# Azure/mmlspark

Measured on NVIDIA H100. Metric: boosting_iters_per_sec, higher is better.
Workload: dtype int64 fixed-point histograms over u8 bins (fp32 gradients, fp64 split gains)

## Files before the change

### mmlspark_b200/csrc/hist_kernel.cuh

```cuda
#pragma once
#include <cstdint>
#include <cuda_runtime.h>
#include <cub/block/block_scan.cuh>

namespace b200gbm {

constexpr int kTileFeat = 32;
constexpr int kBins = 256;
constexpr int kLoBits = 18;
constexpr int kFlushRows = 1 << (32 - kLoBits);
#ifndef B200GBM_K4_EXPERIMENT
#define B200GBM_K4_EXPERIMENT 0
#endif
constexpr int kPlaneWords = kBins * kTileFeat;

struct HistWork {
  int begin;
  int count;
  int use_idx;
  int buf;
};

__global__ void __launch_bounds__(256)
k_gather_q(const HistWork* __restrict__ work, const int* __restrict__ idx0, const int* __restrict__ idx1, const int4* __restrict__ qgh,
           int4* __restrict__ qord) {
  const HistWork w = *work;
  if (!w.use_idx) return;
  const int* __restrict__ idx = w.buf ? idx1 : idx0;
  for (int i = blockIdx.x * blockDim.x + threadIdx.x; i < w.count; i += gridDim.x * blockDim.x) {
    const int p = w.begin + i;
    qord[p] = qgh[idx[p]];
  }
}

constexpr int kBoundBlockRows = 4096;
struct RowBlockBound {
  const int* prefix;
  int blocks;
};
inline int bound_blocks(int num_data) { return (num_data + kBoundBlockRows - 1) / kBoundBlockRows; }

__global__ void __launch_bounds__(256)
k_block_maxcnt(const uint8_t* __restrict__ bins, size_t rows_stride, int num_data, int num_columns, int* __restrict__ prefix) {
  __shared__ unsigned cnt[kBins * kTileFeat];
  __shared__ unsigned wmax[8];
  const int tile = blockIdx.y, tid = threadIdx.x;
  for (int e = tid; e < kBins * kTileFeat; e += blockDim.x) cnt[e] = 0u;
  __syncthreads();
  const int r0 = blockIdx.x * kBoundBlockRows, rows = min(kBoundBlockRows, num_data - r0);
  const unsigned* wp = reinterpret_cast<const unsigned*>(bins + (static_cast<size_t>(tile) * rows_stride + r0) * kTileFeat);
  for (int e = tid; e < rows * 8; e += blockDim.x) {
    const unsigned word = wp[e];
    const int c0 = (e & 7) * 4, rot = (e >> 3) & 3;
#pragma unroll
    for (int k = 0; k < 4; ++k) {
      const int kk = (k + rot) & 3;
      atomicAdd(&cnt[((word >> (8 * kk)) & 0xFFu) * kTileFeat + c0 + kk], 1u);
    }
  }
  __syncthreads();
  const int ncol = min(kTileFeat, num_columns - tile * kTileFeat);
  unsigned m = 0u;
  for (int e = tid; e < kBins * kTileFeat; e += blockDim.x)
    if ((e & (kTileFeat - 1)) < ncol) m = max(m, cnt[e]);
  m = __reduce_max_sync(0xffffffffu, m);
  if ((tid & 31) == 0) wmax[tid >> 5] = m;
  __syncthreads();
  if (tid == 0) {
    for (int i = 1; i < static_cast<int>(blockDim.x >> 5); ++i) m = max(m, wmax[i]);
    prefix[static_cast<size_t>(tile) * (gridDim.x + 1) + blockIdx.x] = static_cast<int>(m);
  }
}

__global__ void __launch_bounds__(1024) k_block_bound_prefix(int blocks, int* __restrict__ prefix) {
  using Scan = cub::BlockScan<int, 1024>;
  __shared__ typename Scan::TempStorage tmp;
  int* p = prefix + static_cast<size_t>(blockIdx.x) * (blocks + 1);
  int carry = 0;
  for (int b0 = 0; b0 < blocks; b0 += 1024) {
    const int b = b0 + threadIdx.x;
    const int v = b < blocks ? p[b] : 0;
    int ex, total;
    Scan(tmp).ExclusiveSum(v, ex, total);
    if (b < blocks) p[b] = carry + ex;
    carry += total;
    __syncthreads();
  }
  if (threadIdx.x == 0) p[blocks] = carry;
}

inline void launch_block_bound(const uint8_t* bins, size_t rows_stride, int num_data, int num_tiles, int num_columns, int* prefix,
                               cudaStream_t stream) {
  const int blocks = bound_blocks(num_data);
  if (blocks > 0) k_block_maxcnt<<<dim3(blocks, num_tiles), 256, 0, stream>>>(bins, rows_stride, num_data, num_columns, prefix);
  k_block_bound_prefix<<<num_tiles, 1024, 0, stream>>>(blocks, prefix);
}


__device__ __forceinline__ void cp_async16(void* smem, const void* gmem, bool valid) {
  unsigned s = static_cast<unsigned>(__cvta_generic_to_shared(smem));
  int sz = valid ? 16 : 0;
  asm volatile("cp.async.cg.shared.global [%0], [%1], 16, %2;\n" ::"r"(s), "l"(gmem), "r"(sz));
}
template <int N>
__device__ __forceinline__ void cp_async_wait() {
  asm volatile("cp.async.wait_group %0;\n" ::"n"(N));
}

constexpr int kWsConsumerWarps = 16;
constexpr int kWsProducerWarps = 2;
constexpr int kWsThreads = (kWsConsumerWarps + kWsProducerWarps) * 32;
constexpr int kWsStageRows = 512;
constexpr int kWsStages = 3;
constexpr int kFlushSlabBins = 32;
constexpr int kFlushRowBytes = kFlushSlabBins * 16;
constexpr int kFlushStageBytes = kTileFeat * kFlushRowBytes;
constexpr int kWsSmemBytes = 4 * kPlaneWords * 4 + kWsStages * (kWsStageRows * 32 + kWsStageRows * 16) + kFlushStageBytes + 64;
static_assert(kWsSmemBytes <= 227 * 1024, "K4 shared memory exceeds the 227 KB per block of sm_90");
static_assert(kFlushSlabBins * kTileFeat == 2 * kWsConsumerWarps * 32, "a flush slab is two (g,h) pairs per consumer thread");

__device__ __forceinline__ unsigned smem_u32(const void* p) { return static_cast<unsigned>(__cvta_generic_to_shared(p)); }
__device__ __forceinline__ void mbar_init(unsigned long long* bar, unsigned count) {
  asm volatile("mbarrier.init.shared::cta.b64 [%0], %1;\n" ::"r"(smem_u32(bar)), "r"(count));
}
__device__ __forceinline__ void mbar_arrive(unsigned long long* bar) {
  asm volatile("mbarrier.arrive.shared::cta.b64 _, [%0];\n" ::"r"(smem_u32(bar)) : "memory");
}
__device__ __forceinline__ void mbar_arrive_expect_tx(unsigned long long* bar, unsigned bytes) {
  asm volatile("mbarrier.arrive.expect_tx.shared::cta.b64 _, [%0], %1;\n" ::"r"(smem_u32(bar)), "r"(bytes) : "memory");
}
__device__ __forceinline__ void mbar_expect_tx(unsigned long long* bar, unsigned bytes) {
  asm volatile("mbarrier.expect_tx.relaxed.cta.shared::cta.b64 [%0], %1;\n" ::"r"(smem_u32(bar)), "r"(bytes) : "memory");
}
__device__ __forceinline__ void mbar_wait(unsigned long long* bar, unsigned parity) {
  asm volatile(
      "{\n"
      ".reg .pred p;\n"
      "WAIT_LOOP:\n"
      "mbarrier.try_wait.parity.shared::cta.b64 p, [%0], %1;\n"
      "@p bra DONE;\n"
      "bra WAIT_LOOP;\n"
      "DONE:\n"
      "}\n" ::"r"(smem_u32(bar)), "r"(parity) : "memory");
}
__device__ __forceinline__ void tma_bulk_g2s(void* smem_dst, const void* gmem_src, unsigned bytes, unsigned long long* bar) {
  asm volatile("cp.async.bulk.shared::cluster.global.mbarrier::complete_tx::bytes [%0], [%1], %2, [%3];\n" ::"r"(smem_u32(smem_dst)),
               "l"(gmem_src), "r"(bytes), "r"(smem_u32(bar))
               : "memory");
}
__device__ __forceinline__ void cp_async_mbar_arrive_noinc(unsigned long long* bar) {
  asm volatile("cp.async.mbarrier.arrive.noinc.shared::cta.b64 [%0];\n" ::"r"(smem_u32(bar)) : "memory");
}
__device__ __forceinline__ void bulk_reduce_add_u64(unsigned long long* gmem_dst, const void* smem_src, unsigned bytes) {
  asm volatile("cp.reduce.async.bulk.global.shared::cta.bulk_group.add.u64 [%0], [%1], %2;\n" ::"l"(gmem_dst), "r"(smem_u32(smem_src)),
               "r"(bytes)
               : "memory");
}
__device__ __forceinline__ void bulk_commit() { asm volatile("cp.async.bulk.commit_group;\n" ::: "memory"); }
__device__ __forceinline__ void bulk_wait_read_all() { asm volatile("cp.async.bulk.wait_group.read 0;\n" ::: "memory"); }
__device__ __forceinline__ void bulk_wait_all() { asm volatile("cp.async.bulk.wait_group 0;\n" ::: "memory"); }
__device__ __forceinline__ void fence_proxy_async_smem() { asm volatile("fence.proxy.async.shared::cta;\n" ::: "memory"); }

template <int NATOM>
__global__ void __launch_bounds__(kWsThreads, 1)
k4_hist_build_ws(const uint8_t* __restrict__ bins, size_t rows_stride, int num_tiles, const int4* __restrict__ qgh,
                 const int4* __restrict__ qord, const int* __restrict__ idx0, const int* __restrict__ idx1,
                 const HistWork* __restrict__ work, unsigned long long* __restrict__ hist, RowBlockBound bound) {
  extern __shared__ __align__(128) unsigned char smem_raw[];
  unsigned* plane = reinterpret_cast<unsigned*>(smem_raw);
  unsigned char* stage_bins = smem_raw + 4 * kPlaneWords * 4;
  int4* stage_q = reinterpret_cast<int4*>(stage_bins + kWsStages * kWsStageRows * 32);
  unsigned char* flush_stage = reinterpret_cast<unsigned char*>(stage_q) + kWsStages * kWsStageRows * 16;
  unsigned long long* full_bar = reinterpret_cast<unsigned long long*>(flush_stage + kFlushStageBytes);
  unsigned long long* empty_bar = full_bar + kWsStages;

  const HistWork w = *work;
  const int n = w.count;
  if (n <= 0) return;
  const int tid = threadIdx.x, lane = tid & 31, warp = tid >> 5;
  const int* __restrict__ idx = w.buf ? idx1 : idx0;

  long long cells_rows = static_cast<long long>(n) * num_tiles;
  int rpi = static_cast<int>((cells_rows + 4LL * gridDim.x - 1) / (4LL * gridDim.x));
  rpi = (rpi + kWsStageRows - 1) / kWsStageRows * kWsStageRows;
  rpi = max(rpi, kWsStageRows);
  rpi = min(rpi, kFlushRows);
  const int chunks = (n + rpi - 1) / rpi;
  const long long items = static_cast<long long>(chunks) * num_tiles;
  const int i0 = static_cast<int>(items * blockIdx.x / gridDim.x);
  const int i1 = static_cast<int>(items * (blockIdx.x + 1) / gridDim.x);
  if (i0 >= i1) return;

  if (tid == 0) {
    for (int i = 0; i < kWsStages; ++i) { mbar_init(&full_bar[i], kWsProducerWarps * 32); mbar_init(&empty_bar[i], kWsConsumerWarps); }
    asm volatile("fence.mbarrier_init.release.cluster;\n" ::: "memory");
  }
  for (int e = tid; e < 4 * kPlaneWords; e += kWsThreads) plane[e] = 0u;
  __syncthreads();

  unsigned gs = 0;
  if (warp >= kWsConsumerWarps) {
    const int ptid = tid - kWsConsumerWarps * 32;
    constexpr int kPT = kWsProducerWarps * 32;
    constexpr int kPerLane = kWsStageRows / kPT;
    for (int item = i0; item < i1; ++item) {
      const int tile = item / chunks, chunk = item - tile * chunks;
      const int row0 = chunk * rpi;
      const int nrows = min(rpi, n - row0);
      const int nst = (nrows + kWsStageRows - 1) / kWsStageRows;
      const uint8_t* tbins = bins + static_cast<size_t>(tile) * rows_stride * 32;
      for (int s = 0; s < nst; ++s, ++gs) {
        const int slot = gs % kWsStages;
        mbar_wait(&empty_bar[slot], ((gs / kWsStages) & 1u) ^ 1u);
        const int p0 = row0 + s * kWsStageRows;
        const int rows = min(kWsStageRows, row0 + nrows - p0);
        unsigned char* db = stage_bins + slot * kWsStageRows * 32;
        int4* dq = stage_q + slot * kWsStageRows;
        if (!w.use_idx) {
          if (ptid == 0) {
            mbar_arrive_expect_tx(&full_bar[slot], static_cast<unsigned>(rows) * 48u);
            const size_t r = static_cast<size_t>(w.begin + p0);
            tma_bulk_g2s(db, tbins + r * 32, static_cast<unsigned>(rows) * 32u, &full_bar[slot]);
            tma_bulk_g2s(dq, qgh + r, static_cast<unsigned>(rows) * 16u, &full_bar[slot]);
          } else {
            mbar_arrive(&full_bar[slot]);
          }
        } else {
          const int* ip = idx + w.begin + p0;
          if (ptid == 0) {
            mbar_expect_tx(&full_bar[slot], static_cast<unsigned>(rows) * 16u);
            tma_bulk_g2s(dq, qord + static_cast<size_t>(w.begin + p0), static_cast<unsigned>(rows) * 16u, &full_bar[slot]);
          }
          int rr[2 * kPerLane];
#pragma unroll
          for (int k = 0; k < 2 * kPerLane; ++k) { const int j = (ptid + k * kPT) >> 1; rr[k] = j < rows ? ip[j] : -1; }
#pragma unroll
          for (int k = 0; k < 2 * kPerLane; ++k) {
            const int hh = ptid + k * kPT, j = hh >> 1, half = (hh & 1) * 16;
            if (rr[k] >= 0) cp_async16(db + j * 32 + half, tbins + static_cast<size_t>(rr[k]) * 32 + half, true);
          }
          cp_async_mbar_arrive_noinc(&full_bar[slot]);
        }
      }
    }
    cp_async_wait<0>();
  } else {
#if B200GBM_K4_EXPERIMENT >= 1 && B200GBM_K4_EXPERIMENT <= 3
    unsigned exp_sink = 0;
#endif
    const int sub = lane >> 2, rot = lane & 3;
    auto item_rows = [&](int it, int& first, int& last) {
      const int t = it / chunks, r0 = (it - t * chunks) * rpi;
      first = w.begin + r0;
      last = first + min(rpi, n - r0) - 1;
      if (w.use_idx && bound.prefix) { first = idx[first]; last = idx[last]; }
    };
    auto item_bound = [&](int it, int first, int last) -> int {
      const int t = it / chunks, nr = min(rpi, n - (it - t * chunks) * rpi);
      if (!bound.prefix) return nr;
      const int* p = bound.prefix + static_cast<size_t>(t) * (bound.blocks + 1);
      return min(nr, p[last / kBoundBlockRows + 1] - p[first / kBoundBlockRows]);
    };
    int first, last;
    item_rows(i0, first, last);
    int next_bound = item_bound(i0, first, last);
    if (i0 + 1 < i1) item_rows(i0 + 1, first, last);
    int acc_bound = 0;
    for (int item = i0; item < i1; ++item) {
      const int tile = item / chunks, chunk = item - tile * chunks;
      const int row0 = chunk * rpi;
      const int nrows = min(rpi, n - row0);
      const int nst = (nrows + kWsStageRows - 1) / kWsStageRows;
      acc_bound += next_bound;
      next_bound = 0;
      if (item + 1 < i1) {
        next_bound = item_bound(item + 1, first, last);
        if (item + 2 < i1) item_rows(item + 2, first, last);
      }
      for (int s = 0; s < nst; ++s, ++gs) {
        const int slot = gs % kWsStages;
        mbar_wait(&full_bar[slot], (gs / kWsStages) & 1u);
        const int rows = min(kWsStageRows, nrows - s * kWsStageRows);
        const unsigned* sw = reinterpret_cast<const unsigned*>(stage_bins + slot * kWsStageRows * 32);
        const int4* sq = stage_q + slot * kWsStageRows;
        const int groups = (rows + 31) >> 5;
        for (int g = warp; g < groups; g += kWsConsumerWarps) {
          const int r = g * 32 + lane;
          if (r < rows) {
            const int4 q = sq[r];
            const unsigned* rw = sw + r * 8;
#pragma unroll
            for (int k = 0; k < 8; ++k) {
              const int w8 = (sub + k) & 7;
              const unsigned word = rw[w8];
#pragma unroll
              for (int j = 0; j < 4; ++j) {
                const int kk = (j + rot) & 3;
                const unsigned b = (word >> (8 * kk)) & 0xFFu;
                const unsigned a = b * 32u + static_cast<unsigned>(w8 * 4 + kk);
#if B200GBM_K4_EXPERIMENT == 0 || B200GBM_K4_EXPERIMENT == 4
                atomicAdd(&plane[a], static_cast<unsigned>(q.x));
                atomicAdd(&plane[kPlaneWords + a], static_cast<unsigned>(q.y));
                atomicAdd(&plane[2 * kPlaneWords + a], static_cast<unsigned>(q.z));
                if (NATOM == 4) atomicAdd(&plane[3 * kPlaneWords + a], static_cast<unsigned>(q.w));
#else
                if (B200GBM_K4_EXPERIMENT >= 2) atomicAdd(&plane[a], static_cast<unsigned>(q.x));
                if (B200GBM_K4_EXPERIMENT >= 3) atomicAdd(&plane[kPlaneWords + a], static_cast<unsigned>(q.y));
                if (B200GBM_K4_EXPERIMENT == 1) exp_sink ^= a + static_cast<unsigned>(q.x ^ q.y ^ q.z ^ q.w);
#endif
              }
            }
          }
        }
#if B200GBM_K4_EXPERIMENT >= 1 && B200GBM_K4_EXPERIMENT <= 3
        if (exp_sink == 0x12345679u) plane[lane] = exp_sink;
#endif
        __syncwarp();
        if (lane == 0) mbar_arrive(&empty_bar[slot]);
      }
      const bool flush = (item + 1 == i1) || ((item + 1) / chunks != tile) || (acc_bound + next_bound > kFlushRows);
      if (!flush) continue;
      acc_bound = 0;
      asm volatile("bar.sync 1, %0;\n" ::"n"(kWsConsumerWarps * 32) : "memory");
      unsigned long long* htile = hist + static_cast<size_t>(tile) * kTileFeat * kBins * 2;
      int sbin[2];
#pragma unroll
      for (int i = 0; i < 2; ++i) sbin[i] = (warp + i * kWsConsumerWarps + lane) & (kFlushSlabBins - 1);
      for (int b0 = 0; b0 < kBins; b0 += kFlushSlabBins) {
        long long g[2], h[2];
        bool nz = false;
#pragma unroll
        for (int i = 0; i < 2; ++i) {
          const int e = (b0 + sbin[i]) * kTileFeat + lane;
          const unsigned ghi = plane[e], glo = plane[kPlaneWords + e], hhi = plane[2 * kPlaneWords + e];
          const unsigned hlo = (NATOM == 4) ? plane[3 * kPlaneWords + e] : 0u;
          plane[e] = 0u;
          plane[kPlaneWords + e] = 0u;
          plane[2 * kPlaneWords + e] = 0u;
          if (NATOM == 4) plane[3 * kPlaneWords + e] = 0u;
          nz |= (ghi | glo | hhi | hlo) != 0u;
          g[i] = (static_cast<long long>(static_cast<int>(ghi)) << kLoBits) + static_cast<long long>(glo);
          h[i] = (NATOM == 4) ? (static_cast<long long>(static_cast<int>(hhi)) << kLoBits) + static_cast<long long>(hlo)
                              : static_cast<long long>(hhi);
        }
        if (tid == 0) bulk_wait_read_all();
        asm volatile("bar.sync 1, %0;\n" ::"n"(kWsConsumerWarps * 32) : "memory");
#pragma unroll
        for (int i = 0; i < 2; ++i)
          *reinterpret_cast<longlong2*>(flush_stage + lane * kFlushRowBytes + sbin[i] * 16) = make_longlong2(g[i], h[i]);
        fence_proxy_async_smem();
        int any;
        asm volatile(
            "{\n"
            ".reg .pred p, q;\n"
            "setp.ne.u32 p, %1, 0;\n"
            "bar.red.or.pred q, 1, %2, p;\n"
            "selp.s32 %0, 1, 0, q;\n"
            "}\n"
            : "=r"(any)
            : "r"(static_cast<unsigned>(nz)), "n"(kWsConsumerWarps * 32)
            : "memory");
#if B200GBM_K4_EXPERIMENT != 4
        if (tid == 0 && any) {
          for (int f = 0; f < kTileFeat; ++f)
            bulk_reduce_add_u64(htile + (static_cast<size_t>(f) * kBins + b0) * 2, flush_stage + f * kFlushRowBytes, kFlushSlabBins * 16);
          bulk_commit();
        }
#else
        (void)any; (void)htile;
#endif
      }
    }
    if (tid == 0) bulk_wait_all();
  }
}

inline cudaError_t set_k4_smem_limit() {
  const cudaError_t e = cudaFuncSetAttribute(k4_hist_build_ws<4>, cudaFuncAttributeMaxDynamicSharedMemorySize, kWsSmemBytes);
  if (e != cudaSuccess) return e;
  return cudaFuncSetAttribute(k4_hist_build_ws<3>, cudaFuncAttributeMaxDynamicSharedMemorySize, kWsSmemBytes);
}

inline void launch_k4(bool const_hessian, const uint8_t* bins, size_t rows_stride, int num_tiles, const int4* qgh, const int4* qord,
                      const int* idx0, const int* idx1, const HistWork* work, unsigned long long* hist, RowBlockBound bound, int grid,
                      cudaStream_t stream) {
  if (const_hessian)
    k4_hist_build_ws<3><<<grid, kWsThreads, kWsSmemBytes, stream>>>(bins, rows_stride, num_tiles, qgh, qord, idx0, idx1, work, hist, bound);
  else
    k4_hist_build_ws<4><<<grid, kWsThreads, kWsSmemBytes, stream>>>(bins, rows_stride, num_tiles, qgh, qord, idx0, idx1, work, hist, bound);
}

}
```

Measured before the change: 6.325.

## Band CTAs by row range across tiles and add L2 evict-first hints on bin loads

Work assignment in the warp-specialized histogram kernel changes: when each CTA has enough rows, CTAs are grouped into row bands so that all feature tiles for a row range are processed together by a set of CTAs. This keeps the shared gradient/hessian rows hot in L2 across tiles. Bin loads (TMA bulk and cp.async) now carry an L2 evict_first cache policy so streamed bin bytes do not displace the reused gradient data. An experiment-5 path that aliases the gradient source is also added behind a macro that is off by default. The new partitioning adds index math and may worsen load balance for tail CTAs.

```diff
diff --git a/mmlspark_b200/csrc/hist_kernel.cuh b/mmlspark_b200/csrc/hist_kernel.cuh
--- a/mmlspark_b200/csrc/hist_kernel.cuh
+++ b/mmlspark_b200/csrc/hist_kernel.cuh
@@ -97,10 +97,14 @@
 }
 
 
-__device__ __forceinline__ void cp_async16(void* smem, const void* gmem, bool valid) {
+__device__ __forceinline__ unsigned long long l2_evict_first_policy() {
+  unsigned long long p;
+  asm volatile("createpolicy.fractional.L2::evict_first.b64 %0, 1.0;\n" : "=l"(p));
+  return p;
+}
+__device__ __forceinline__ void cp_async16(void* smem, const void* gmem, unsigned long long l2_policy) {
   unsigned s = static_cast<unsigned>(__cvta_generic_to_shared(smem));
-  int sz = valid ? 16 : 0;
-  asm volatile("cp.async.cg.shared.global [%0], [%1], 16, %2;\n" ::"r"(s), "l"(gmem), "r"(sz));
+  asm volatile("cp.async.cg.shared.global.L2::cache_hint [%0], [%1], 16, %2;\n" ::"r"(s), "l"(gmem), "l"(l2_policy));
 }
 template <int N>
 __device__ __forceinline__ void cp_async_wait() {
@@ -146,6 +150,12 @@
 __device__ __forceinline__ void tma_bulk_g2s(void* smem_dst, const void* gmem_src, unsigned bytes, unsigned long long* bar) {
   asm volatile("cp.async.bulk.shared::cluster.global.mbarrier::complete_tx::bytes [%0], [%1], %2, [%3];\n" ::"r"(smem_u32(smem_dst)),
                "l"(gmem_src), "r"(bytes), "r"(smem_u32(bar))
+               : "memory");
+}
+__device__ __forceinline__ void tma_bulk_g2s_hint(void* smem_dst, const void* gmem_src, unsigned bytes, unsigned long long* bar,
+                                                  unsigned long long l2_policy) {
+  asm volatile("cp.async.bulk.shared::cluster.global.mbarrier::complete_tx::bytes.L2::cache_hint [%0], [%1], %2, [%3], %4;\n"
+               ::"r"(smem_u32(smem_dst)), "l"(gmem_src), "r"(bytes), "r"(smem_u32(bar)), "l"(l2_policy)
                : "memory");
 }
 __device__ __forceinline__ void cp_async_mbar_arrive_noinc(unsigned long long* bar) {
@@ -180,16 +190,42 @@
   const int tid = threadIdx.x, lane = tid & 31, warp = tid >> 5;
   const int* __restrict__ idx = w.buf ? idx1 : idx0;
 
-  long long cells_rows = static_cast<long long>(n) * num_tiles;
-  int rpi = static_cast<int>((cells_rows + 4LL * gridDim.x - 1) / (4LL * gridDim.x));
+  const int num_ctas = static_cast<int>(gridDim.x), band_ctas = num_ctas / num_tiles * num_tiles;
+  const long long per_cta = static_cast<long long>(n) * num_tiles / num_ctas;
+  int seg_begin = 0, seg_end = n, seg_ctas = num_ctas, seg_cta = blockIdx.x;
+  if (band_ctas > 0 && per_cta >= kFlushRows) {
+    const int bands = band_ctas / num_tiles;
+    const bool tail = band_ctas < num_ctas;
+    const long long band_rows = tail ? per_cta : (n + bands - 1LL) / bands;
+    const int nb = tail ? static_cast<int>(bands * band_rows) : n;
+    if (seg_cta < band_ctas) {
+      const int r = seg_cta / num_tiles;
+      seg_begin = static_cast<int>(min(r * band_rows, static_cast<long long>(nb)));
+      seg_end = static_cast<int>(min(seg_begin + band_rows, static_cast<long long>(nb)));
+      seg_ctas = num_tiles;
+      seg_cta -= r * num_tiles;
+    } else {
+      seg_begin = nb;
+      seg_ctas = num_ctas - band_ctas;
+      seg_cta -= band_ctas;
+    }
+  }
+  const int seg_rows = seg_end - seg_begin;
+  const long long cells_rows = static_cast<long long>(seg_rows) * num_tiles;
+  int rpi = static_cast<int>((cells_rows + 4LL * seg_ctas - 1) / (4LL * seg_ctas));
   rpi = (rpi + kWsStageRows - 1) / kWsStageRows * kWsStageRows;
   rpi = max(rpi, kWsStageRows);
   rpi = min(rpi, kFlushRows);
-  const int chunks = (n + rpi - 1) / rpi;
+  const int chunks = (seg_rows + rpi - 1) / rpi;
   const long long items = static_cast<long long>(chunks) * num_tiles;
-  const int i0 = static_cast<int>(items * blockIdx.x / gridDim.x);
-  const int i1 = static_cast<int>(items * (blockIdx.x + 1) / gridDim.x);
+  const int i0 = static_cast<int>(items * seg_cta / seg_ctas);
+  const int i1 = static_cast<int>(items * (seg_cta + 1) / seg_ctas);
   if (i0 >= i1) return;
+  auto item_span = [&](int it, int& tile, int& row0, int& nrows) {
+    tile = it / chunks;
+    row0 = seg_begin + (it - tile * chunks) * rpi;
+    nrows = min(rpi, seg_end - row0);
+  };
 
   if (tid == 0) {
     for (int i = 0; i < kWsStages; ++i) { mbar_init(&full_bar[i], kWsProducerWarps * 32); mbar_init(&empty_bar[i], kWsConsumerWarps); }
@@ -203,10 +239,10 @@
     const int ptid = tid - kWsConsumerWarps * 32;
     constexpr int kPT = kWsProducerWarps * 32;
     constexpr int kPerLane = kWsStageRows / kPT;
+    const unsigned long long bins_policy = l2_evict_first_policy();
     for (int item = i0; item < i1; ++item) {
-      const int tile = item / chunks, chunk = item - tile * chunks;
-      const int row0 = chunk * rpi;
-      const int nrows = min(rpi, n - row0);
+      int tile, row0, nrows;
+      item_span(item, tile, row0, nrows);
       const int nst = (nrows + kWsStageRows - 1) / kWsStageRows;
       const uint8_t* tbins = bins + static_cast<size_t>(tile) * rows_stride * 32;
       for (int s = 0; s < nst; ++s, ++gs) {
@@ -220,8 +256,12 @@
           if (ptid == 0) {
             mbar_arrive_expect_tx(&full_bar[slot], static_cast<unsigned>(rows) * 48u);
             const size_t r = static_cast<size_t>(w.begin + p0);
-            tma_bulk_g2s(db, tbins + r * 32, static_cast<unsigned>(rows) * 32u, &full_bar[slot]);
+            tma_bulk_g2s_hint(db, tbins + r * 32, static_cast<unsigned>(rows) * 32u, &full_bar[slot], bins_policy);
+#if B200GBM_K4_EXPERIMENT == 5
+            tma_bulk_g2s(dq, qgh + (p0 & 65535), static_cast<unsigned>(rows) * 16u, &full_bar[slot]);
+#else
             tma_bulk_g2s(dq, qgh + r, static_cast<unsigned>(rows) * 16u, &full_bar[slot]);
+#endif
           } else {
             mbar_arrive(&full_bar[slot]);
           }
@@ -229,7 +269,11 @@
           const int* ip = idx + w.begin + p0;
           if (ptid == 0) {
             mbar_expect_tx(&full_bar[slot], static_cast<unsigned>(rows) * 16u);
+#if B200GBM_K4_EXPERIMENT == 5
+            tma_bulk_g2s(dq, qord + (p0 & 65535), static_cast<unsigned>(rows) * 16u, &full_bar[slot]);
+#else
             tma_bulk_g2s(dq, qord + static_cast<size_t>(w.begin + p0), static_cast<unsigned>(rows) * 16u, &full_bar[slot]);
+#endif
           }
           int rr[2 * kPerLane];
 #pragma unroll
@@ -237,7 +281,7 @@
 #pragma unroll
           for (int k = 0; k < 2 * kPerLane; ++k) {
             const int hh = ptid + k * kPT, j = hh >> 1, half = (hh & 1) * 16;
-            if (rr[k] >= 0) cp_async16(db + j * 32 + half, tbins + static_cast<size_t>(rr[k]) * 32 + half, true);
+            if (rr[k] >= 0) cp_async16(db + j * 32 + half, tbins + static_cast<size_t>(rr[k]) * 32 + half, bins_policy);
           }
           cp_async_mbar_arrive_noinc(&full_bar[slot]);
         }
@@ -250,13 +294,15 @@
 #endif
     const int sub = lane >> 2, rot = lane & 3;
     auto item_rows = [&](int it, int& first, int& last) {
-      const int t = it / chunks, r0 = (it - t * chunks) * rpi;
+      int t, r0, nr;
+      item_span(it, t, r0, nr);
       first = w.begin + r0;
-      last = first + min(rpi, n - r0) - 1;
+      last = first + nr - 1;
       if (w.use_idx && bound.prefix) { first = idx[first]; last = idx[last]; }
     };
     auto item_bound = [&](int it, int first, int last) -> int {
-      const int t = it / chunks, nr = min(rpi, n - (it - t * chunks) * rpi);
+      int t, r0, nr;
+      item_span(it, t, r0, nr);
       if (!bound.prefix) return nr;
       const int* p = bound.prefix + static_cast<size_t>(t) * (bound.blocks + 1);
       return min(nr, p[last / kBoundBlockRows + 1] - p[first / kBoundBlockRows]);
@@ -267,9 +313,8 @@
     if (i0 + 1 < i1) item_rows(i0 + 1, first, last);
     int acc_bound = 0;
     for (int item = i0; item < i1; ++item) {
-      const int tile = item / chunks, chunk = item - tile * chunks;
-      const int row0 = chunk * rpi;
-      const int nrows = min(rpi, n - row0);
+      int tile, row0, nrows;
+      item_span(item, tile, row0, nrows);
       const int nst = (nrows + kWsStageRows - 1) / kWsStageRows;
       acc_bound += next_bound;
       next_bound = 0;
@@ -298,7 +343,7 @@
                 const int kk = (j + rot) & 3;
                 const unsigned b = (word >> (8 * kk)) & 0xFFu;
                 const unsigned a = b * 32u + static_cast<unsigned>(w8 * 4 + kk);
-#if B200GBM_K4_EXPERIMENT == 0 || B200GBM_K4_EXPERIMENT == 4
+#if B200GBM_K4_EXPERIMENT == 0 || B200GBM_K4_EXPERIMENT >= 4
                 atomicAdd(&plane[a], static_cast<unsigned>(q.x));
                 atomicAdd(&plane[kPlaneWords + a], static_cast<unsigned>(q.y));
                 atomicAdd(&plane[2 * kPlaneWords + a], static_cast<unsigned>(q.z));
```

New measurement: 6.449 (median of 6 runs). 1.02x the previous value.
